# janstenner/DistributedConvRL-PDE-Control

Measured on AMD Instinct MI355X. Metric: env-steps/sec (KS CNAB2 env step + conv actor fwd + DDPG fwd/bwd/update), higher is better.
Workload: dtype f32

## Files before the change

distributedconvrl-pde-control_amd/_lib.py:

```python
import ctypes as C
import os

_HERE = os.path.dirname(os.path.abspath(__file__))
LIB_PATH = os.environ.get("PDEC_LIB_PATH") or os.path.join(_HERE, "libpdeconv.so")

PDEC_F32, PDEC_F64 = 0, 1
PDE_KS_CNAB2, PDE_KSEG_RK4, PDE_KS_RK4_FD, PDE_FLUID_RK4, PDE_KSEG2D_RK4 = 0, 1, 2, 3, 4
ACT_IDENTITY, ACT_RELU, ACT_TANH = 0, 1, 2

Handle = C.c_uint64


class PdecError(RuntimeError):
    pass


class EnvCfg(C.Structure):
    _fields_ = [
        ("pde_kind", C.c_int), ("dtype", C.c_int), ("B", C.c_int), ("N", C.c_int),
        ("n_species", C.c_int), ("S", C.c_int), ("A", C.c_int), ("window", C.c_int),
        ("temporal_steps", C.c_int), ("mono", C.c_int), ("K", C.c_int), ("check_max_value", C.c_int),
        ("Lx", C.c_double), ("dt", C.c_double), ("mu", C.c_double), ("max_value", C.c_double),
        ("sensor_scale", C.c_double), ("agent_power", C.c_double), ("reward_in_scale", C.c_double),
        ("reward_offset", C.c_double), ("reward_power", C.c_double), ("reward_denom", C.c_double),
# ... 99 lines not shown
    "pdec_ledger_eval_close": [Handle, _vp, _vp, _i64, _i64, _i64],
    "pdec_ledger_eval_read": [Handle, _vp, _vp, _vp, _vp], "pdec_ledger_eval_best": [Handle, _pd, C.POINTER(_i64)],
    "pdec_ledger_eval_best_params": [Handle, Handle],
    "pdec_epclock_create": [C.POINTER(Handle), Handle, _i, _i, _i, _u64, _i, _i], "pdec_epclock_set": [Handle, _vp],
    "pdec_epclock_step": [Handle] + [_vp] * 9, "pdec_epclock_read": [Handle, _vp, _vp, _vp, _vp, _vp],
    "pdec_nstep_create": [C.POINTER(Handle), _i, _i, _i, _i, _i],
    "pdec_nstep_step": [Handle, _vp, _vp, _vp, _vp, _d, _vp, _vp, _vp, _vp], "pdec_nstep_read": [Handle, C.POINTER(_i64)] + [_vp] * 4,
    "pdec_telemetry_create": [C.POINTER(Handle), _i, _i, _i, _i, _i, _i, Handle, Handle],
    "pdec_telemetry_step": [Handle, _vp, _vp, _vp, _vp, _vp, _d], "pdec_telemetry_update": [Handle] * 5 + [_vp],
    "pdec_telemetry_read": [Handle, _vp, C.POINTER(_i64), _vp, C.POINTER(_i64), _vp], "pdec_telemetry_reset": [Handle],
    "pdec_capture_begin": [Handle], "pdec_capture_end": [Handle, C.POINTER(Handle)],
    "pdec_graph_launch": [Handle, _vp], "pdec_graph_num_nodes": [Handle, C.POINTER(_i)],
    "pdec_event_create": [C.POINTER(Handle)], "pdec_event_record": [Handle, _vp], "pdec_stream_wait_event": [_vp, Handle], "pdec_mlp_set_stop_event": [Handle, Handle], "pdec_mlp_flush_stop_event": [Handle],
    "pdec_mlp_set_reduce_event": [Handle, Handle],
    "pdec_env_set_simd_sharing": [Handle, C.c_int, C.POINTER(C.c_int)],
    "pdec_ddpg_critic_grads": [Handle] * 4 + [_vp] * 5 + [_i, _d, _i, _d, _vp],
    "pdec_ddpg_actor_grads": [Handle, Handle, _vp, _i, _d, _vp],
    "pdec_ddpg_update": [Handle] * 4 + [_vp] * 5 + [_i, _d, _d, _i, _d, _d, _pd, _pd],
    "pdec_comm_unique_id": [_vp], "pdec_comm_create": [C.POINTER(Handle), _i, _i, _vp],
    "pdec_comm_create_timeout": [C.POINTER(Handle), _i, _i, _vp, _i],
    "pdec_allreduce_grads": [Handle, Handle], "pdec_allreduce": [Handle, _vp, _sz, _i, _vp],
    "pdec_allreduce_grads_on": [Handle, Handle, _vp],
}
DEBUG_SIGNATURES = {
    "pdec_debug_wave_fft": [_vp, _vp, _i, _i, _i],
    "pdec_debug_wave_fft_f32": [_vp, _vp, _i, _i, _i],
    "pdec_debug_critic_stamps": [Handle, _i, _pd],
    "pdec_debug_fused_image": [Handle, _i, _vp] + [C.POINTER(_i)] * 4,
    "pdec_debug_kseg2d_probe": [Handle, _i, _i, _i, _pd],
    "pdec_debug_spin_us": [_vp, _d],
# ... 150 lines not shown
```

distributedconvrl-pde-control_amd/csrc/env.hip:

```cpp
#include "env_sense.hpp"
#include "roll_actor.hpp"

namespace pdec {

template <class T, int MODE, bool FLT = false>
__global__ void sense_kernel(EnvArg<T, FLT> e, const T* __restrict__ y, const T* __restrict__ action,
                             const T* __restrict__ action_prev, const T* __restrict__ state_prev,
                             T* __restrict__ out) {
  sense_traj<T, MODE, FLT>(e, blockIdx.x, y, action, action_prev, state_prev, out);
}

template <class T>
__global__ void terminal_from_done_kernel(const int32_t* __restrict__ done, int B, int cpt, T* __restrict__ term) {
  const int i = blockIdx.x * blockDim.x + threadIdx.x;
  if (i < B * cpt) term[i] = (done[i / cpt] & 1) ? (T)1 : (T)0;
}

static int launch_step(Env& E, int mode, const StepArgs& a) {
  const pdec_env_cfg& c = E.cfg;
  const bool fused = mode == 0;
  const LaunchSync sync = E.sync;
  E.sync = LaunchSync{};
  if (sync.wait || sync.done) {
    const bool ok = c.pde_kind == PDEC_PDE_KS_CNAB2 && fused && c.B <= 2 && !E.member && c.dtype == PDEC_F64 && ks_is_fixed_plan(E.engine) &&
// ... 265 lines not shown
  }

int pdec_env_set_terminal_out(pdec_handle h, void* terminal_per_column) {
  GET_ENV(E, h);
  E->term_out = terminal_per_column;
  return PDEC_OK;
}

int pdec_env_set_simd_sharing(pdec_handle h, int on, int* effective) {
  GET_ENV(E, h);
  E->share_simd = on != 0;
  if (effective) *effective = (E->share_simd && E->cfg.pde_kind == PDEC_PDE_KS_CNAB2 && ks_is_single_wave(E->engine) && E->cfg.dtype == PDEC_F32) ? 1 : 0;
  return PDEC_OK;
}

int pdec_env_set_member_layout(pdec_handle h, int on) {
  GET_ENV(E, h);
  const int k = E->cfg.pde_kind;
  PDEC_REQUIRE(!on || k == PDEC_PDE_KS_CNAB2 || k == PDEC_PDE_KSEG_RK4,
               "pdec_env_set_member_layout: the 1-D KS and Keller-Segel environments only (pde kind %d)", k);
  PDEC_REQUIRE(!on || !E->rsum_out, "pdec_env_set_member_layout: per-pair reward partials are set (pdec_env_set_reward_partials_out)");
  E->member = on != 0;
  return PDEC_OK;
}

int pdec_env_set_disturbance(pdec_handle h, const void* mu_per_trajectory) {
  GET_ENV(E, h);
  const pdec_env_cfg& c = E->cfg;
  if (mu_per_trajectory) {
    PDEC_REQUIRE(c.pde_kind != PDEC_PDE_FLUID_RK4, "pdec_env_set_disturbance: the fluid has no disturbance term (KS environments only)");
// ... 174 lines not shown
```

distributedconvrl-pde-control_amd/csrc/env.hpp:

```cpp
#pragma once
#include "common.hpp"
#include "fft_lds.hpp"
#include <type_traits>

namespace pdec {

template <class T>
struct EnvDev {
  int B, N, S, A, ns, window, temporal, mono, K, check_max, n_species, rk2, prio;
  int mem, na;
  T sensor_scale, agent_power, r_in_scale, r_offset, r_power, r_denom, a_pun, da_pun, max_value;
  T dx, hstep, dist_mu;
  const T* Gs;
  const int* sn0;
  const T* GaC;
  const int* an0;
  int Wd, Cnt;
  float* rsum_out;
  T* term_out;
  const T* gsum;
  const int* a2s;
  const int* fmap;
  const T *c1, *c2, *c3, *c4, *g;
  const C2<T>* dhat;
// ... 13 lines not shown
struct EnvDevF : EnvDev<T> {
  FaultDev<T> flt;
};
template <class T, bool FLT>
using EnvArg = std::conditional_t<FLT, EnvDevF<T>, EnvDev<T>>;

enum class KsEngine {
  Wave256,
  Wave1024,
  LdsR4_256,
  LdsR4_1024,
  Fixed192,
  Fixed240,
  Fixed600,
  Generic,
};
constexpr bool ks_is_single_wave(KsEngine k) { return k == KsEngine::Wave256; }
constexpr bool ks_is_fixed_plan(KsEngine k) { return k == KsEngine::Fixed192 || k == KsEngine::Fixed240 || k == KsEngine::Fixed600; }
inline KsEngine ks_pick_engine(int N, bool force_generic, bool lds_fft) {
  if (force_generic) return KsEngine::Generic;
  if (N == 256) return lds_fft ? KsEngine::LdsR4_256 : KsEngine::Wave256;
  if (N == 1024) return lds_fft ? KsEngine::LdsR4_1024 : KsEngine::Wave1024;
  return N == 192 ? KsEngine::Fixed192 : N == 240 ? KsEngine::Fixed240 : N == 600 ? KsEngine::Fixed600 : KsEngine::Generic;
}
int ks_engine_threads(KsEngine k);

struct StepArgs {
  const void *y_in, *p, *action, *action_prev, *state_prev;
  void *y_out, *p_out, *state_out, *reward_out;
  int32_t* done;
};

struct Env : Object {
  pdec_env_cfg cfg;
  DevBuf Gs, sn0, GaC, an0, gsum, a2s, fmap, c1, c2, c3, c4, g, dhat, dhat1, tw;
  int Wd = 0, Cnt = 0;
  DevBuf stage;
  DevBuf roll;
  DevBuf roll_tab;
  std::vector<const void*> roll_tab_host;
  DevBuf mem_scratch;
  void* term_out = nullptr;
  float* rsum_out = nullptr;
  bool share_simd = false;
  bool member = false;
  const void* mu_b = nullptr;
  int control_from = 0;
  const void *act_gain = nullptr, *sens_gain = nullptr, *sens_bias = nullptr;
  bool faults() const { return act_gain || sens_gain || sens_bias; }
  FftPlan fft;
  int nthreads = 64;
  KsEngine engine = KsEngine::Generic;
  size_t lds_bytes = 0;
  Env() : Object(Kind::Env) {}
  virtual int part_streams() const { return 0; }
  virtual int set_part_streams(const hipStream_t*, int) { return PDEC_OK; }
  virtual int actuate(const void* action, void* p_out);
  virtual int featurize(const void* y, const void* state_prev, void* state_out, const void* action = nullptr);
  virtual int reward(const void* y, const void* action, const void* action_prev, void* r_out);
  virtual int pde_step(const void* y_in, const void* p, void* y_out, int32_t* done);
  virtual int rhs_eval(const void* y, const void* p, void* out);
  virtual int env_step(const StepArgs& a);
};

template <class T>
EnvDev<T> make_dev(const Env& E) {
  const pdec_env_cfg& c = E.cfg;
  EnvDev<T> e;
  e.B = c.B; e.N = c.N; e.S = c.S; e.A = c.A; e.window = c.window; e.temporal = c.temporal_steps;
  e.mono = c.mono; e.K = c.K; e.check_max = c.check_max_value; e.n_species = c.n_species;
  e.mem = c.memory_size; e.na = 1 + c.memory_size;
  e.ns = c.mono ? c.S : c.window * c.n_species * c.temporal_steps + c.memory_size;
  e.sensor_scale = (T)c.sensor_scale; e.agent_power = (T)c.agent_power;
  e.r_in_scale = (T)c.reward_in_scale; e.r_offset = (T)c.reward_offset; e.r_power = (T)c.reward_power;
  e.r_denom = (T)c.reward_denom; e.a_pun = (T)c.action_punish; e.da_pun = (T)c.delta_action_punish;
  e.max_value = (T)c.max_value;
  e.dx = (T)(c.Lx / c.N);
  e.hstep = (T)(c.dt / c.K);
// ... 92 lines not shown
```

distributedconvrl-pde-control_amd/csrc/env_sense.hpp:

```cpp
#pragma once
#include "env.hpp"

namespace pdec {


template <class T, class YF>
__device__ __forceinline__ void sense_dots(const EnvDev<T>& e, YF yf, T* dots, T* part, int tid, int nt) {
  const int S = e.S, N = e.N, Wd = e.Wd;
  int ng = nt / S;
  if (ng < 1) ng = 1;
  if (ng > 8) ng = 8;
  const int chunk = (Wd + ng - 1) / ng;
  for (int idx = tid; idx < ng * S; idx += nt) {
    const int grp = idx / S, s = idx - grp * S;
    int j0 = grp * chunk, j1 = j0 + chunk;
    if (j1 > Wd) j1 = Wd;
    int n = e.sn0[s] + j0;
    if (n >= N) n -= N;
    T p0[4] = {0, 0, 0, 0}, p1[4] = {0, 0, 0, 0};
    int j = j0;
    for (; j + 8 <= j1; j += 8) {
      T gk[8];
#pragma unroll
      for (int u = 0; u < 8; ++u) gk[u] = e.Gs[(size_t)(j + u) * S + s];
// ... 325 lines not shown
```

distributedconvrl-pde-control_amd/csrc/ks_engines.hpp:

```cpp
#pragma once
#include "env.hpp"

namespace pdec {

#define KS_MPT 4

template <class T>
struct FftGeneric {
  static constexpr int kThreads = 1024;
  C2<T>*X, *Y;
  const C2<T>* tw;
  FftPlan pl;
  int N, tid, nt;
  __device__ __forceinline__ void init(unsigned char* smem, const EnvDev<T>& e, int tid_, int nt_) {
    N = e.N; tid = tid_; nt = nt_; pl = e.fft;
    X = reinterpret_cast<C2<T>*>(smem);
    Y = X + N;
    C2<T>* t = Y + N;
    for (int k = tid; k < N; k += nt) t[k] = e.tw[k];
    tw = t;
  }
  static __host__ __device__ size_t lds_complex(int N) { return 3 * (size_t)N; }
  __device__ __forceinline__ int mode_index(int j) const { return tid + j * nt; }
  __device__ __forceinline__ int phys_index(int j) const { return tid + j * nt; }
// ... 276 lines not shown
      dft4<+1>(a);
      exchange<2>(a); twiddle<2, +1>(a); dft4<+1>(a);
      exchange<1>(a); twiddle<1, +1>(a); dft4<+1>(a);
      exchange<0>(a); twiddle<0, +1>(a); dft4<+1>(a);
    }
  }
  __device__ __forceinline__ C2<T>* publish(const C2<T> (&a)[KS_MPT]) {
    __syncthreads();
#pragma unroll
    for (int j = 0; j < 4; ++j) buf[tid + NT * j] = a[j];
    __syncthreads();
    return buf;
  }
};

template <class T>
struct FftWave1024 {
  static constexpr int kThreads = 256;
  static constexpr int N = 1024, NT = 256;
  FftWave256<T> core;
  C2<T>* buf[2];
  C2<T> wx[3];
  int tid, lane, wv, par;
  __device__ __forceinline__ void init(unsigned char* smem, const EnvDev<T>& e, int tid_, int) {
    tid = tid_; lane = tid & 63; wv = tid >> 6; par = 0;
    buf[0] = reinterpret_cast<C2<T>*>(smem);
    buf[1] = buf[0] + N;
    core.tid = lane;
    core.b1 = (lane & 2) != 0; core.b0 = (lane & 1) != 0;
    core.buf = buf[0];
// ... 122 lines not shown
  __device__ __forceinline__ C2<T>* publish(const C2<T> (&a)[KS_MPT]) {
    __syncthreads();
#pragma unroll
    for (int j = 0; j < KS_MPT; ++j) {
      const int k = phys_index(j);
      if (k < N) buf[0][k] = a[j];
    }
    __syncthreads();
    return buf[0];
  }
};
template <class T> using FftFixed192 = FftFixed<T, 192, 4, 4, 4, 3, 4, 1>;
template <class T> using FftFixed240 = FftFixed<T, 240, 4, 4, 5, 3, 4, 1>;
template <class T> using FftFixed600 = FftFixed<T, 600, 5, 4, 5, 5, 2, 3>;

template <KsEngine K, class ENG> struct KsEngineTag { static constexpr KsEngine kind = K; using type = ENG; };
template <class T, class F>
auto with_ks_engine(KsEngine k, F&& f) {
  switch (k) {
    case KsEngine::Wave256: return f(KsEngineTag<KsEngine::Wave256, FftWave256<T>>{});
    case KsEngine::Wave1024: return f(KsEngineTag<KsEngine::Wave1024, FftWave1024<T>>{});
    case KsEngine::LdsR4_256: return f(KsEngineTag<KsEngine::LdsR4_256, FftR4<T, 4>>{});
    case KsEngine::LdsR4_1024: return f(KsEngineTag<KsEngine::LdsR4_1024, FftR4<T, 5>>{});
    case KsEngine::Fixed192: return f(KsEngineTag<KsEngine::Fixed192, FftFixed192<T>>{});
    case KsEngine::Fixed240: return f(KsEngineTag<KsEngine::Fixed240, FftFixed240<T>>{});
    case KsEngine::Fixed600: return f(KsEngineTag<KsEngine::Fixed600, FftFixed600<T>>{});
    default: return f(KsEngineTag<KsEngine::Generic, FftGeneric<T>>{});
  }
}

}
```

distributedconvrl-pde-control_amd/csrc/ks_step.hip:

```cpp
#include "env_sense.hpp"
#include "ks_engines.hpp"

namespace pdec {

template <class T, class ENG, bool FUSED, bool SHARE = false, bool SYNC = false, bool MU = false, bool FLT = false>
__global__ void __launch_bounds__(ENG::kThreads, SHARE ? 8 : 1) ks_env_step_kernel(EnvArg<T, FLT> e, const T* __restrict__ y_in, const T* __restrict__ p_in,
                                   const T* __restrict__ action, const T* __restrict__ action_prev,
                                   const T* __restrict__ state_prev, T* __restrict__ y_out,
                                   T* __restrict__ p_out, T* __restrict__ state_out,
                                   T* __restrict__ reward_out, int32_t* __restrict__ done) {
  extern __shared__ __align__(16) unsigned char smem_raw[];
  const int N = e.N, tid = threadIdx.x, nt = blockDim.x;
  if constexpr (SYNC) launch_sync_wait(e.sync);
  set_wave_prio(e.prio);
  ENG eng;
  eng.init(smem_raw, e, tid, nt);
  T* act = reinterpret_cast<T*>(reinterpret_cast<C2<T>*>(smem_raw) + ENG::lds_complex(N));
  T* actp = act + 2 * e.A;
  T* dots = actp + 2 * e.A;
  T* part = dots + 2 * e.S;
  T* red = part + 16 * e.S;

  const int b0 = e.member ? (int)blockIdx.x : 2 * (int)blockIdx.x, b1 = b0 + 1;
  const bool has1 = !e.member && b1 < e.B;
  const size_t o0 = (size_t)b0 * N, o1 = (size_t)b1 * N;
  const C2<T>* __restrict__ dtab = MU ? e.dhat1 : e.dhat;
  T m0 = 1, m1 = 1;
// ... 4 lines not shown
      act[a] = action[(size_t)b0 * e.A + a];
      act[e.A + a] = has1 ? action[(size_t)b1 * e.A + a] : (T)0;
      actp[a] = action_prev[(size_t)b0 * e.A + a];
      actp[e.A + a] = has1 ? action_prev[(size_t)b1 * e.A + a] : (T)0;
      if constexpr (FLT) {
        act[a] = fault_action<T>(e.flt, b0, e.A, a, act[a]);
        if (has1) act[e.A + a] = fault_action<T>(e.flt, b1, e.A, a, act[e.A + a]);
      }
    }
  }
  __syncthreads();

  constexpr bool LDSC = SHARE;
  typedef T T4v __attribute__((ext_vector_type(4)));
  T4v* cst = reinterpret_cast<T4v*>(smem_raw + ((size_t)(reinterpret_cast<unsigned char*>(red + 16) - smem_raw + 15) & ~(size_t)15));
  C2<T> U[KS_MPT], Nn[KS_MPT], Ck[KS_MPT], v[KS_MPT];
  T kc1[KS_MPT], kc2[KS_MPT], kc3[KS_MPT], kg[KS_MPT];
  T pa4[KS_MPT], pb4[KS_MPT];
  if (FUSED) {
    int n4[KS_MPT];
#pragma unroll
    for (int j = 0; j < KS_MPT; ++j) n4[j] = eng.phys_index(j);
    if ((N & 3) == 0 && 2 * N <= 16 * e.S) {
      actuate_consecutive<T>(e, act, act + e.A, part, tid, nt);
#pragma unroll
      for (int j = 0; j < KS_MPT; ++j) {
        pa4[j] = n4[j] < N ? part[n4[j]] : (T)0;
        pb4[j] = n4[j] < N ? part[N + n4[j]] : (T)0;
      }
    } else {
      actuate_cells<T, KS_MPT>(e, act, act + e.A, n4, pa4, pb4);
    }
    if constexpr (FLT) {
      __syncthreads();
      for (int a = tid; a < e.A; a += nt) {
        act[a] = action[(size_t)b0 * e.A + a];
        if (has1) act[e.A + a] = action[(size_t)b1 * e.A + a];
      }
    }
  }
#pragma unroll
  for (int j = 0; j < KS_MPT; ++j) {
    const int n = eng.phys_index(j);
    T pa = 0, pb = 0;
    if (n < N) {
      if (FUSED) {
        pa = pa4[j]; pb = pb4[j];
        if (!has1) pb = 0;
        if (p_out) {
          p_out[o0 + n] = pa;
          if (has1) p_out[o1 + n] = pb;
        }
      } else {
        pa = p_in[o0 + n];
        pb = has1 ? p_in[o1 + n] : (T)0;
      }
    }
    v[j] = mk<T>(pa, pb);
  }
  eng.template run<-1>(v);
#pragma unroll
  for (int j = 0; j < KS_MPT; ++j) {
    const int k = eng.mode_index(j);
    if (k < N) {
      const C2<T> d = dtab[k];
      const T c4 = e.c4[k];
      if constexpr (MU) Ck[j] = mk<T>(c4 * v[j].x + (m0 * d.x - m1 * d.y), c4 * v[j].y + (m0 * d.y + m1 * d.x));
      else Ck[j] = mk<T>(c4 * v[j].x + (d.x - d.y), c4 * v[j].y + (d.x + d.y));
      kc1[j] = e.c1[k];
      kc2[j] = e.c2[k];
      kc3[j] = e.c3[k];
      kg[j] = e.g[k];
    } else {
      Ck[j] = mk<T>(0, 0);
      kc1[j] = kc2[j] = kc3[j] = kg[j] = 0;
    }
    if constexpr (LDSC) cst[j * nt + tid] = T4v{kc1[j], kc2[j], kc3[j], kg[j]};
  }
  if constexpr (LDSC) {
    cst[4 * nt + tid] = T4v{Ck[0].x, Ck[0].y, Ck[1].x, Ck[1].y};
    cst[5 * nt + tid] = T4v{Ck[2].x, Ck[2].y, Ck[3].x, Ck[3].y};
  }
#pragma unroll
  for (int j = 0; j < KS_MPT; ++j) {
    const int n = eng.phys_index(j);
    U[j] = n < N ? mk<T>(y_in[o0 + n], has1 ? y_in[o1 + n] : (T)0) : mk<T>(0, 0);
    v[j] = mk<T>(U[j].x * U[j].x, U[j].y * U[j].y);
  }
  eng.template run<-1>(v);
#pragma unroll
  for (int j = 0; j < KS_MPT; ++j) Nn[j] = cscale(mul_i<+1, T>(v[j]), kg[j]);
  if constexpr (LDSC) {
    cst[6 * nt + tid] = T4v{Nn[0].x, Nn[0].y, Nn[1].x, Nn[1].y};
    cst[7 * nt + tid] = T4v{Nn[2].x, Nn[2].y, Nn[3].x, Nn[3].y};
  }
  eng.template run<-1>(U);
  const T invN = (T)1 / (T)N;
  if constexpr (LDSC) {
    for (int it = 0; it < e.K; ++it) {
#pragma unroll
      for (int j = 0; j < KS_MPT; ++j) v[j] = U[j];
      eng.template run<+1>(v);
#pragma unroll
      for (int j = 0; j < KS_MPT; ++j) {
        const T wr = v[j].x * invN, wi = v[j].y * invN;
        v[j] = mk<T>(wr * wr, wi * wi);
      }
      eng.template run<-1>(v);
#pragma unroll
      for (int h = 0; h < 2; ++h) {
        const T4v nn = cst[(6 + h) * nt + tid], ck = cst[(4 + h) * nt + tid];
        T4v nw;
#pragma unroll
        for (int u = 0; u < 2; ++u) {
          const int j = 2 * h + u;
          const T4v c = cst[j * nt + tid];
          const C2<T> n1 = cscale(mul_i<+1, T>(v[j]), c[3]);
          U[j] = mk<T>(c[0] * U[j].x + c[1] * n1.x - c[2] * nn[2 * u] + ck[2 * u],
                       c[0] * U[j].y + c[1] * n1.y - c[2] * nn[2 * u + 1] + ck[2 * u + 1]);
          nw[2 * u] = n1.x; nw[2 * u + 1] = n1.y;
        }
        cst[(6 + h) * nt + tid] = nw;
      }
    }
  } else {
    for (int it = 0; it < e.K; ++it) {
#pragma unroll
      for (int j = 0; j < KS_MPT; ++j) v[j] = U[j];
      eng.template run<+1>(v);
#pragma unroll
      for (int j = 0; j < KS_MPT; ++j) {
        const T wr = v[j].x * invN, wi = v[j].y * invN;
        v[j] = mk<T>(wr * wr, wi * wi);
      }
      eng.template run<-1>(v);
#pragma unroll
      for (int j = 0; j < KS_MPT; ++j) {
        const C2<T> nn1 = Nn[j];
        Nn[j] = cscale(mul_i<+1, T>(v[j]), kg[j]);
        U[j] = mk<T>(kc1[j] * U[j].x + kc2[j] * Nn[j].x - kc3[j] * nn1.x + Ck[j].x,
                     kc1[j] * U[j].y + kc2[j] * Nn[j].y - kc3[j] * nn1.y + Ck[j].y);
      }
    }
  }
  eng.template run<+1>(U);
  T mx0 = 0, mx1 = 0;
#pragma unroll
  for (int j = 0; j < KS_MPT; ++j) {
    const int n = eng.phys_index(j);
    U[j] = mk<T>(U[j].x * invN, U[j].y * invN);
    if (n < N) {
      y_out[o0 + n] = U[j].x;
      if (has1) y_out[o1 + n] = U[j].y;
      if (!(fabs(U[j].x) <= e.max_value)) mx0 = 1;
      if (!(fabs(U[j].y) <= e.max_value)) mx1 = 1;
    }
  }
  if (done) {
    mx0 = block_max<T>(mx0, red, tid, nt);
    mx1 = block_max<T>(mx1, red, tid, nt);
    if (tid == 0) {
      const bool chk = e.check_max == 1;
      done[b0] = (chk && mx0 > 0) ? 1 : 0;
      if (has1) done[b1] = (chk && mx1 > 0) ? 1 : 0;
    }
    if (FUSED && e.check_max != 2) {
      write_terminal<T>(e, b0, e.check_max == 1 && mx0 > 0, tid, nt);
      if (has1) write_terminal<T>(e, b1, e.check_max == 1 && mx1 > 0, tid, nt);
    }
  }
  if (!FUSED) return;
  const T* Rt = reinterpret_cast<const T*>(eng.publish(U));
  sense_dots<T>(e, [&](int r, int n) { return Rt[2 * n + r]; }, dots, part, tid, nt);
  const int rw = e.mono ? 1 : e.A;
  const int sw = e.mono ? e.S : e.A * e.ns;
  T rmine;
  const T* fd = dots;
  if constexpr (FLT) {
    fault_dots<T>(e.flt, b0, e.S, dots, part, tid, nt);
    if (has1) fault_dots<T>(e.flt, b1, e.S, dots + e.S, part + e.S, tid, nt);
    __syncthreads();
    fd = part;
  }
  if (e.fmap && !e.mono) {
    rmine = reward_pair<T>(e, dots, dots + e.S, act, act + e.A, actp, actp + e.A, reward_out + (size_t)b0 * rw,
                           has1 ? reward_out + (size_t)b1 * rw : nullptr, tid, nt);
    featurize_pair<T>(e, fd, fd + e.S, state_out + (size_t)b0 * sw, has1 ? state_out + (size_t)b1 * sw : nullptr, tid, nt);
  } else {
    rmine = reward_traj<T>(e, dots, act, actp, reward_out + (size_t)b0 * rw, tid, nt);
    featurize_traj<T>(e, fd, state_prev ? state_prev + (size_t)b0 * sw : nullptr, state_out + (size_t)b0 * sw, tid, nt);
    if (has1) {
      rmine += reward_traj<T>(e, dots + e.S, act + e.A, actp + e.A, reward_out + (size_t)b1 * rw, tid, nt);
      featurize_traj<T>(e, fd + e.S, state_prev ? state_prev + (size_t)b1 * sw : nullptr,
                        state_out + (size_t)b1 * sw, tid, nt);
    }
  }
  if (e.rsum_out) {
    float v = (float)rmine;
    for (int off = 32; off > 0; off >>= 1) v += __shfl_xor(v, off);
    __syncthreads();
    if ((tid & 63) == 0) red[tid >> 6] = (T)v;
    __syncthreads();
    if (tid == 0) {
      float tot = 0.f;
      for (int i = 0; i < (nt + 63) / 64; ++i) tot += (float)red[i];
      e.rsum_out[blockIdx.x] = tot;
    }
// ... 3 lines not shown
    if (tid == 0) {
      for (int t = 0; t < (has1 ? 2 : 1); ++t) {
        T m = 0;
        const T* r = reward_out + (size_t)(b0 + t) * rw;
        for (int a = 0; a < rw; ++a)
          if (!(fabs(r[a]) <= e.max_value)) m = 1;
        done[b0 + t] = m > 0 ? 1 : 0;
        write_terminal<T>(e, b0 + t, m > 0, 0, 1);
      }
    }
  }
  if constexpr (SYNC) launch_sync_done(e.sync);
}

int ks_engine_threads(KsEngine k) {
  return with_ks_engine<float>(k, [](auto tag) { return (int)decltype(tag)::type::kThreads; });
}
size_t ks_lds_bytes(const pdec_env_cfg& c, KsEngine k) {
  const size_t fft = with_ks_engine<float>(k, [&](auto tag) { return decltype(tag)::type::lds_complex(c.N); });
  return (fft * 2 + 4 * (size_t)c.A + 2 * c.S + 16 * c.S + 16) * dtype_size(c.dtype);
}

template <class T, class ENG, KsEngine KIND, bool FLT>
auto ks_step_kernel_for(bool fused, bool share, bool synced, bool mu) {
  auto kern = mu ? ks_env_step_kernel<T, ENG, true, false, false, true, FLT> : ks_env_step_kernel<T, ENG, true, false, false, false, FLT>;
  if constexpr (!FLT)
    if (!fused) kern = mu ? ks_env_step_kernel<T, ENG, false, false, false, true> : ks_env_step_kernel<T, ENG, false>;
  if constexpr (sizeof(T) == 4 && ks_is_single_wave(KIND))
    if (share) kern = mu ? ks_env_step_kernel<T, ENG, true, true, false, true, FLT> : ks_env_step_kernel<T, ENG, true, true, false, false, FLT>;
  if constexpr (!FLT && sizeof(T) == 8 && ks_is_fixed_plan(KIND))
    if (synced) kern = mu ? ks_env_step_kernel<T, ENG, true, false, true, true> : ks_env_step_kernel<T, ENG, true, false, true>;
  return kern;
}

int ks_launch_step(Env& E, bool fused, const StepArgs& a, const LaunchSync& sync) {
  const pdec_env_cfg& c = E.cfg;
  const dim3 grid(E.member ? c.B : (c.B + 1) / 2), block(E.nthreads);
  const bool synced = sync.wait || sync.done;
  const bool mu = E.mu_b != nullptr;
  const bool share = fused && E.share_simd && c.dtype == PDEC_F32 && ks_is_single_wave(E.engine);
  const size_t lds = E.lds_bytes + (share ? 16 + 8 * 16 * 64 : 0);
  const bool timed = c.dtype == PDEC_F32 && ks_is_single_wave(E.engine) && fused && E.prof && E.prof_reps == 1;
  by_dtype(c.dtype, [&](auto t) {
    using T = decltype(t);
    with_ks_engine<T>(E.engine, [&](auto tag) {
      using ENG = typename decltype(tag)::type;
      constexpr KsEngine KIND = decltype(tag)::kind;
      auto launch = [&](auto kern, const auto& e) {
        if (timed) {
          PDEC_TIMED_LAUNCH(&E, "ks_env_step", kern, grid, block, lds, PDEC_STEP_KERNEL_ARGS(T, e, a));
          return;
        }
        ProfScope ps(&E, fused ? "ks_env_step" : "ks_pde_step", !synced && a.y_out != a.y_in && a.state_out != a.state_prev);
        for (int rep = 0; rep < ps.reps; ++rep) hipLaunchKernelGGL(kern, grid, block, lds, E.stream, PDEC_STEP_KERNEL_ARGS(T, e, a));
      };
      if (fused && E.faults()) {
        launch(ks_step_kernel_for<T, ENG, KIND, true>(fused, share, synced, mu), make_dev_faults<T>(E));
      } else {
        EnvDev<T> e = make_dev<T>(E);
        e.sync = sync;
        launch(ks_step_kernel_for<T, ENG, KIND, false>(fused, share, synced, mu), e);
      }
    });
  });
  PDEC_HIP(hipGetLastError());
  return PDEC_OK;
}

}
```

distributedconvrl-pde-control_amd/env.py:

```python
import ctypes as C

import numpy as np
import torch

from . import _lib


def _stream_ptr(stream):
    if stream is None:
        return None
    return C.c_void_p(stream.cuda_stream)


_FAST_STREAM_SWITCH = hasattr(torch._C, "_cuda_getCurrentStream") and hasattr(torch._C, "_cuda_setStream")


class _on_stream:
    __slots__ = ("s", "prev", "ctx")

    def __init__(self, stream):
        self.s, self.prev, self.ctx = stream, None, None

    def __enter__(self):
        s = self.s
# ... 290 lines not shown
        self.time += self.dt
        self._done_stale = True
        if self.autoreset:
            own_action = self.action.data_ptr() not in self._adopted
            _lib.check(self.lib.pdec_env_autoreset(
                self._h, _lib.ptr(self._done_flags), _lib.ptr(self.y), _lib.ptr(self.y0), _lib.ptr(self.state),
                _lib.ptr(self._state0), _lib.ptr(self.action) if own_action else None,
                _lib.ptr(self.action0) if own_action else None, _lib.ptr(self.reward)))

    def set_simd_sharing(self, on=True):
        import ctypes as C
        eff = C.c_int()
        _lib.check(self.lib.pdec_env_set_simd_sharing(self.handle, 1 if on else 0, C.byref(eff)))
        return bool(eff.value)

    def set_disturbance(self, mu):
        if mu is None:
            _lib.check(self.lib.pdec_env_set_disturbance(self._h, None))
            self.mu = None
            return
        with _on_stream(self.stream):
            t = mu if isinstance(mu, torch.Tensor) else torch.as_tensor(np.array(mu, dtype=np.float64, copy=True))
            if t.dim() != 1 or int(t.shape[0]) != self.B:
                raise _lib.PdecError(f"PDEenv.set_disturbance: expected {self.B} amplitudes (one per trajectory), got shape "
                                     f"{tuple(t.shape)}")
            t = t.to(device=self.device, dtype=self.dtype).contiguous().clone()
        _lib.check(self.lib.pdec_env_set_disturbance(self._h, _lib.ptr(t)))
        self.mu = t

    def set_faults(self, actuator_gain=None, sensor_gain=None, sensor_bias=None):
# ... 98 lines not shown
```

distributedconvrl-pde-control_amd/pipeline.py:

```python
import copy
import ctypes as C
import os
from types import SimpleNamespace

import torch

from . import _lib
from .pipeline_episodes import check_episode_mode, setup_episodes
from .pipeline_eval import Evaluation, check_eval_args, eval_score
from .pipeline_nstep import NStep, check_n_step, gamma_n
from .pipeline_replay import Replay
from .pipeline_telemetry import (TELEMETRY_STEP_COLUMNS, TELEMETRY_UPDATE_COLUMNS, Telemetry, check_telemetry,
                                 ring_columns)

PERIOD = 6


class _Event(_lib.Owned):

    def __init__(self, lib):
        super().__init__(lib)
        _lib.check(lib.pdec_event_create(C.byref(self.h)))

    def record(self, stream):
# ... 121 lines not shown
        self.actor = self.policy.behavior_actor.model
        yes = C.c_int()
        _lib.check(self.lib.pdec_mlp_acts_on_published_copy(self.actor.handle, C.byref(yes)))
        self.act_in_place = not bool(yes.value)
        self.kick_env_after_critic = ((not self.act_in_place and not self.use_replay) if kick_env_after_critic is None
                                      else bool(kick_env_after_critic))
        if os.environ.get("PDEC_KICK") in ("0", "1"):
            self.kick_env_after_critic = os.environ["PDEC_KICK"] == "1"
        self.stop_events = (self.rpart is not None and Ev is _Event and not self.serial
                            and os.environ.get("PDEC_STOP_EVENTS", "1") != "0")
        self.simd_sharing = False
        if not self.serial and self.rpart is not None and os.environ.get("PDEC_SHARE", "0") == "1":
            eff = C.c_int()
            _lib.check(self.lib.pdec_env_set_simd_sharing(env.handle, 1, C.byref(eff)))
            self.simd_sharing = bool(eff.value)
        self.graphs = {}
        self._progs = {}
        aliases = (self.policy.behavior_critic.model.dtype == torch.float32) if self.use_replay else self._batch_aliases
        self.fast_eager = os.environ.get("PDEC_FAST_EAGER", "1") == "1" and Ev is _Event and aliases
        self._key, self._captured = None, False
        self.n_graph_launches = self.n_eager_steps = 0
        self.noise_scale = None
        self.set_noise_scale(noise_scale)
        self.noise_ab = self.noise_state = None
        self.set_noise_corr(noise_corr)
        self.nstep = NStep(self) if self.n_step > 1 else None
        self._telem = Telemetry(self) if self.telemetry_capacity > 0 else None
        self.replay = Replay(self) if self.use_replay else None
        self.ledger, self.inits, self.clock = setup_episodes(self, log_episodes, min_best_episode, random_init, init_seed, init_rng,
                                                             init_rank)
# ... 551 lines not shown
    def telemetry_reset(self):
        self._on("_telem", "TrainPipeline.telemetry_reset: telemetry is off (telemetry=0)").reset()

    def sync(self):
        self._flush_actor_finish()
        for s in (self.s_env, self.s_upd, self.s_ar, self.s_eval):
            if s is not None:
                s.synchronize()

    def close(self):
        if self.s_eval is not None:
            self.s_eval.synchronize()
        if getattr(self, "simd_sharing", False):
            self.lib.pdec_env_set_simd_sharing(self.env.handle, 0, None)
            self.simd_sharing = False
        self._drop_graphs()
```

include/pdeconv.h:

```cpp
#ifndef PDECONV_H
#define PDECONV_H

#include <stddef.h>
#include <stdint.h>

#ifdef __cplusplus
extern "C" {
#endif

typedef uint64_t pdec_handle;

enum { PDEC_F32 = 0, PDEC_F64 = 1 };

enum {
  PDEC_OK = 0,
  PDEC_E_INVALID = -1,
  PDEC_E_HIP = -2,
  PDEC_E_HANDLE = -3,
  PDEC_E_NOGPU = -4,
  PDEC_E_COMM = -5
};

enum {
  PDEC_PDE_KS_CNAB2 = 0,
// ... 156 lines not shown
                     double* actor_loss, double* critic_loss);

int pdec_ddpg_update_async(pdec_handle A, pdec_handle C, pdec_handle At, pdec_handle Ct,
                           const void* s, const void* a, const void* r, const void* t, const void* snext,
                           int Bu, double gamma, double rho, int quirk, double eta_actor, double eta_critic,
                           void* losses_dev);

int pdec_ddpg_update_small(pdec_handle A, pdec_handle C, pdec_handle At, pdec_handle Ct,
                           const void* state_trace, const void* action_trace, const void* reward_trace,
                           const void* terminal_trace, const int32_t* idx_s, const int32_t* idx_rt,
                           const int32_t* idx_sn, int loops, int Bu, double gamma, double rho, int quirk,
                           double eta_actor, double eta_critic, void* losses_dev);

int pdec_reward_mean(pdec_handle any_handle, const void* r, int n, void* mean_out);
int pdec_env_set_simd_sharing(pdec_handle env, int on, int* effective);
int pdec_env_set_reward_partials_out(pdec_handle env, void* partial_sums, int* n_partials);
int pdec_env_part_streams(pdec_handle env, int* n);
int pdec_env_set_part_streams(pdec_handle env, void* const* hip_streams, int n);
int pdec_ddpg_set_reward_partials(pdec_handle critic, const void* partial_sums, int n);
int pdec_ddpg_set_reward_mean(pdec_handle critic, const void* mean_dev);

int pdec_ddpg_set_reward_groups(pdec_handle critic, int g, int L);

int pdec_ddpg_update_small_rng(pdec_handle A, pdec_handle C, pdec_handle At, pdec_handle Ct,
                               const void* state_trace, const void* action_trace, const void* reward_trace,
                               const void* terminal_trace, int loops, int Bu, uint64_t seed, uint64_t offset,
                               int64_t n_valid, int64_t n_rt, int64_t capacity, int stride, double gamma, double rho,
                               int quirk, double eta_actor, double eta_critic, void* losses_dev);

int pdec_ddpg_update_critic_async(pdec_handle A, pdec_handle C, pdec_handle At, pdec_handle Ct,
// ... 114 lines not shown
```

Before: 4.933 million.

## Add two-wave 256-point FFT engine for the fused KS CNAB2 env step

Adds a new FFT engine, Wave256x2, that splits the 256-point KS FFT across two wavefronts of 64 lanes (128 threads, 2 modes per thread). One butterfly level exchanges data across the two waves through LDS with a barrier, and the remaining levels use intra-wave DPP and permlane swaps. It is enabled by default in the pipeline for the fused f32 step when SIMD sharing is off. Reward and sense reductions are limited to the first 64 threads. The aim is to halve per-thread register work and the serial FFT latency of each env-step block, at the cost of extra LDS round trips and cross-wave barriers inside every FFT.

```diff
diff --git a/distributedconvrl-pde-control_amd/_lib.py b/distributedconvrl-pde-control_amd/_lib.py
--- a/distributedconvrl-pde-control_amd/_lib.py
+++ b/distributedconvrl-pde-control_amd/_lib.py
@@ -137,6 +137,7 @@
     "pdec_event_create": [C.POINTER(Handle)], "pdec_event_record": [Handle, _vp], "pdec_stream_wait_event": [_vp, Handle], "pdec_mlp_set_stop_event": [Handle, Handle], "pdec_mlp_flush_stop_event": [Handle],
     "pdec_mlp_set_reduce_event": [Handle, Handle],
     "pdec_env_set_simd_sharing": [Handle, C.c_int, C.POINTER(C.c_int)],
+    "pdec_env_set_two_wave_step": [Handle, C.c_int, C.POINTER(C.c_int)],
     "pdec_ddpg_critic_grads": [Handle] * 4 + [_vp] * 5 + [_i, _d, _i, _d, _vp],
     "pdec_ddpg_actor_grads": [Handle, Handle, _vp, _i, _d, _vp],
     "pdec_ddpg_update": [Handle] * 4 + [_vp] * 5 + [_i, _d, _d, _i, _d, _d, _pd, _pd],
diff --git a/distributedconvrl-pde-control_amd/csrc/env.hip b/distributedconvrl-pde-control_amd/csrc/env.hip
--- a/distributedconvrl-pde-control_amd/csrc/env.hip
+++ b/distributedconvrl-pde-control_amd/csrc/env.hip
@@ -303,6 +303,13 @@
   return PDEC_OK;
 }
 
+int pdec_env_set_two_wave_step(pdec_handle h, int on, int* effective) {
+  GET_ENV(E, h);
+  E->two_wave = on != 0;
+  if (effective) *effective = ks_step_engine(*E, true) == KsEngine::Wave256x2 ? 1 : 0;
+  return PDEC_OK;
+}
+
 int pdec_env_set_member_layout(pdec_handle h, int on) {
   GET_ENV(E, h);
   const int k = E->cfg.pde_kind;
diff --git a/distributedconvrl-pde-control_amd/csrc/env.hpp b/distributedconvrl-pde-control_amd/csrc/env.hpp
--- a/distributedconvrl-pde-control_amd/csrc/env.hpp
+++ b/distributedconvrl-pde-control_amd/csrc/env.hpp
@@ -51,6 +51,7 @@
   Fixed240,
   Fixed600,
   Generic,
+  Wave256x2,
 };
 constexpr bool ks_is_single_wave(KsEngine k) { return k == KsEngine::Wave256; }
 constexpr bool ks_is_fixed_plan(KsEngine k) { return k == KsEngine::Fixed192 || k == KsEngine::Fixed240 || k == KsEngine::Fixed600; }
@@ -80,6 +81,7 @@
   void* term_out = nullptr;
   float* rsum_out = nullptr;
   bool share_simd = false;
+  bool two_wave = false;
   bool member = false;
   const void* mu_b = nullptr;
   int control_from = 0;
@@ -99,6 +101,12 @@
   virtual int rhs_eval(const void* y, const void* p, void* out);
   virtual int env_step(const StepArgs& a);
 };
+
+inline KsEngine ks_step_engine(const Env& E, bool fused) {
+  const bool two = E.two_wave && fused && E.cfg.pde_kind == PDEC_PDE_KS_CNAB2 && E.engine == KsEngine::Wave256 &&
+                   E.cfg.dtype == PDEC_F32 && !E.share_simd && !E.member && !E.mu_b && !E.faults();
+  return two ? KsEngine::Wave256x2 : E.engine;
+}
 
 template <class T>
 EnvDev<T> make_dev(const Env& E) {
diff --git a/distributedconvrl-pde-control_amd/csrc/env_sense.hpp b/distributedconvrl-pde-control_amd/csrc/env_sense.hpp
--- a/distributedconvrl-pde-control_amd/csrc/env_sense.hpp
+++ b/distributedconvrl-pde-control_amd/csrc/env_sense.hpp
@@ -3,6 +3,7 @@
 
 namespace pdec {
 
+constexpr int SUM_IDLE_TID = 1 << 28;
 
 template <class T, class YF>
 __device__ __forceinline__ void sense_dots(const EnvDev<T>& e, YF yf, T* dots, T* part, int tid, int nt) {
diff --git a/distributedconvrl-pde-control_amd/csrc/ks_engines.hpp b/distributedconvrl-pde-control_amd/csrc/ks_engines.hpp
--- a/distributedconvrl-pde-control_amd/csrc/ks_engines.hpp
+++ b/distributedconvrl-pde-control_amd/csrc/ks_engines.hpp
@@ -314,6 +314,158 @@
   }
 };
 
+__device__ __forceinline__ void wave_pair_barrier() { asm volatile("s_waitcnt lgkmcnt(0)\n\ts_barrier" ::: "memory"); }
+#define PDEC_XSTEP2(CA, CB, MASK, P0, Q0, P1, Q1)                                                          \
+  {                                                                                                        \
+    float n0_, n1_;                                                                                        \
+    asm("s_nop 1\n\t"                                                                                      \
+        "s_mov_b64 vcc, %6\n\t"                                                                            \
+        "v_cndmask_b32_dpp %4, %0, %1, vcc " CA " row_mask:0xf bank_mask:0xf\n\t"                           \
+        "v_cndmask_b32_dpp %5, %2, %3, vcc " CA " row_mask:0xf bank_mask:0xf\n\t"                           \
+        "s_mov_b64 vcc, %7\n\t"                                                                            \
+        "v_cndmask_b32_dpp %0, %1, %0, vcc " CB " row_mask:0xf bank_mask:0xf\n\t"                           \
+        "v_cndmask_b32_dpp %2, %3, %2, vcc " CB " row_mask:0xf bank_mask:0xf"                                \
+        : "+v"(P0), "+v"(Q0), "+v"(P1), "+v"(Q1), "=&v"(n0_), "=&v"(n1_)                                   \
+        : "s"(MASK), "s"(~(MASK))                                                                          \
+        : "vcc");                                                                                          \
+    Q0 = n0_; Q1 = n1_;                                                                                    \
+  }
+template <int SGN>
+__device__ __forceinline__ pkf2 pk_cmul_lanes(pkf2 a, pkf2 w, unsigned long long mask) {
+  pkf2 t;
+  unsigned long long sv;
+  if (SGN < 0)
+    asm("s_and_saveexec_b64 %2, %4\n\t"
+        "v_pk_mul_f32 %1, %0, %3 op_sel_hi:[1,0]\n\t"
+        "v_pk_fma_f32 %0, %0, %3, %1 op_sel:[1,1,0] op_sel_hi:[0,1,1] neg_lo:[0,1,0]\n\t"
+        "s_mov_b64 exec, %2"
+        : "+v"(a), "=&v"(t), "=&s"(sv) : "v"(w), "s"(mask) : "scc");
+  else
+    asm("s_and_saveexec_b64 %2, %4\n\t"
+        "v_pk_mul_f32 %1, %0, %3 op_sel_hi:[1,0]\n\t"
+        "v_pk_fma_f32 %0, %0, %3, %1 op_sel:[1,1,0] op_sel_hi:[0,1,1] neg_hi:[0,1,0]\n\t"
+        "s_mov_b64 exec, %2"
+        : "+v"(a), "=&v"(t), "=&s"(sv) : "v"(w), "s"(mask) : "scc");
+  return a;
+}
+
+struct FftWave256x2 {
+  static constexpr int kThreads = 128;
+  static constexpr int kMpt = 2;
+  static constexpr int kSumThreads = 64;
+  static constexpr int N = 256, NT = 128;
+  C2<float>* buf;
+  pkf2 w0[3], w1[3];
+  int tid, lane, wv, par;
+  __device__ __forceinline__ void init(unsigned char* smem, const EnvDev<float>& e, int tid_, int) {
+    tid = tid_; lane = tid & 63; par = 0;
+    wv = __builtin_amdgcn_readfirstlane(tid >> 6);
+    buf = reinterpret_cast<C2<float>*>(smem);
+    const int kl[3] = {wv, (lane >> 4) & 1, (lane >> 2) & 1};
+    const int low[3] = {lane, 4 * (lane & 15), 16 * (lane & 3)};
+#pragma unroll
+    for (int st = 0; st < 3; ++st) {
+      w0[st] = __builtin_bit_cast(pkf2, e.tw[(kl[st] * low[st]) & 255]);
+      w1[st] = __builtin_bit_cast(pkf2, e.tw[((kl[st] + 2) * low[st]) & 255]);
+    }
+  }
+  static __host__ __device__ size_t lds_complex(int) { return (size_t)N; }
+  __device__ __forceinline__ int mode_index(int j) const {
+    const int k0 = wv + 2 * (lane >> 5), k1 = ((lane >> 4) & 1) + 2 * ((lane >> 3) & 1);
+    const int k2 = ((lane >> 2) & 1) + 2 * ((lane >> 1) & 1), k3 = (lane & 1) + 2 * j;
+    return k0 + 4 * k1 + 16 * k2 + 64 * k3;
+  }
+  __device__ __forceinline__ int phys_index(int j) const { return tid + NT * j; }
+
+  static __device__ __forceinline__ void level1(C2<float> (&a)[2]) {
+    const pkf2 p = __builtin_bit_cast(pkf2, a[0]), q = __builtin_bit_cast(pkf2, a[1]);
+    a[0] = __builtin_bit_cast(C2<float>, p + q);
+    a[1] = __builtin_bit_cast(C2<float>, p - q);
+  }
+  template <int SGN>
+  static __device__ __forceinline__ void level2(C2<float> (&a)[2], bool d) {
+    const C2<float> b = a[1];
+    pkf2 r;
+    if (SGN < 0) { r.x = d ? b.y : b.x; r.y = d ? -b.x : b.y; }
+    else { r.x = d ? -b.y : b.x; r.y = d ? b.x : b.y; }
+    const pkf2 p = __builtin_bit_cast(pkf2, a[0]);
+    a[0] = __builtin_bit_cast(C2<float>, p + r);
+    a[1] = __builtin_bit_cast(C2<float>, p - r);
+  }
+  template <int SGN>
+  __device__ __forceinline__ void level2_wave(C2<float> (&a)[2]) const {
+    const pkf2 p = __builtin_bit_cast(pkf2, a[0]), q = __builtin_bit_cast(pkf2, a[1]);
+    if (wv) {
+      a[0] = __builtin_bit_cast(C2<float>, SGN < 0 ? pk_add_mi(p, q) : pk_add_pi(p, q));
+      a[1] = __builtin_bit_cast(C2<float>, SGN < 0 ? pk_add_pi(p, q) : pk_add_mi(p, q));
+    } else {
+      a[0] = __builtin_bit_cast(C2<float>, p + q);
+      a[1] = __builtin_bit_cast(C2<float>, p - q);
+    }
+  }
+  template <int ST, int SGN>
+  __device__ __forceinline__ void twiddle(C2<float> (&a)[2]) const {
+    a[1] = __builtin_bit_cast(C2<float>, pk_cmul<SGN>(__builtin_bit_cast(pkf2, a[1]), w1[ST]));
+    if (ST == 0) {
+      if (wv) a[0] = __builtin_bit_cast(C2<float>, pk_cmul<SGN>(__builtin_bit_cast(pkf2, a[0]), w0[0]));
+    } else {
+      a[0] = __builtin_bit_cast(C2<float>, pk_cmul_lanes<SGN>(__builtin_bit_cast(pkf2, a[0]), w0[ST],
+                                                              ST == 1 ? 0xFFFF0000FFFF0000ull : 0xF0F0F0F0F0F0F0F0ull));
+    }
+  }
+  template <int BIT>
+  static __device__ __forceinline__ void xch(C2<float> (&a)[2]) {
+    if (BIT == 5) {
+      asm("s_nop 1\n\t"
+          "v_permlane32_swap_b32 %0, %2\n\t"
+          "v_permlane32_swap_b32 %1, %3"
+          : "+v"(a[0].x), "+v"(a[0].y), "+v"(a[1].x), "+v"(a[1].y));
+    } else if (BIT == 4) {
+      asm("s_nop 1\n\t"
+          "v_permlane16_swap_b32 %0, %2\n\t"
+          "v_permlane16_swap_b32 %1, %3"
+          : "+v"(a[0].x), "+v"(a[0].y), "+v"(a[1].x), "+v"(a[1].y));
+    } else if (BIT == 3) {
+      PDEC_XSTEP2("row_ror:8", "row_ror:8", 0xFF00FF00FF00FF00ull, a[0].x, a[1].x, a[0].y, a[1].y)
+    } else if (BIT == 2) {
+      PDEC_XSTEP2("row_ror:12", "row_ror:4", 0xF0F0F0F0F0F0F0F0ull, a[0].x, a[1].x, a[0].y, a[1].y)
+    } else if (BIT == 1) {
+      PDEC_XSTEP2("quad_perm:[2,3,0,1]", "quad_perm:[2,3,0,1]", 0xCCCCCCCCCCCCCCCCull, a[0].x, a[1].x, a[0].y, a[1].y)
+    } else {
+      PDEC_XSTEP2("quad_perm:[1,0,3,2]", "quad_perm:[1,0,3,2]", 0xAAAAAAAAAAAAAAAAull, a[0].x, a[1].x, a[0].y, a[1].y)
+    }
+  }
+  __device__ __forceinline__ void xch_wave(C2<float> (&a)[2]) {
+    C2<float>* X = buf + 128 * par;
+    par ^= 1;
+    if (wv) X[tid] = a[0]; else X[tid] = a[1];
+    wave_pair_barrier();
+    if (wv) a[0] = X[tid ^ 64]; else a[1] = X[tid ^ 64];
+  }
+  template <int SGN>
+  __device__ __forceinline__ void run(C2<float> (&a)[2]) {
+    const bool d4 = (lane & 16) != 0, d2 = (lane & 4) != 0, d0 = (lane & 1) != 0;
+    if (SGN < 0) {
+      level1(a); xch_wave(a); level2_wave<-1>(a); twiddle<0, -1>(a);
+      xch<5>(a); level1(a); xch<4>(a); level2<-1>(a, d4); twiddle<1, -1>(a);
+      xch<3>(a); level1(a); xch<2>(a); level2<-1>(a, d2); twiddle<2, -1>(a);
+      xch<1>(a); level1(a); xch<0>(a); level2<-1>(a, d0);
+    } else {
+      level1(a); xch<0>(a); level2<+1>(a, d0);
+      xch<1>(a); twiddle<2, +1>(a); level1(a); xch<2>(a); level2<+1>(a, d2);
+      xch<3>(a); twiddle<1, +1>(a); level1(a); xch<4>(a); level2<+1>(a, d4);
+      xch<5>(a); twiddle<0, +1>(a); level1(a); xch_wave(a); level2_wave<+1>(a);
+    }
+  }
+  __device__ __forceinline__ C2<float>* publish(const C2<float> (&a)[2]) {
+    __syncthreads();
+#pragma unroll
+    for (int j = 0; j < 2; ++j) buf[tid + NT * j] = a[j];
+    __syncthreads();
+    return buf;
+  }
+};
+
 template <class T>
 struct FftWave1024 {
   static constexpr int kThreads = 256;
@@ -466,9 +618,16 @@
 template <class T> using FftFixed240 = FftFixed<T, 240, 4, 4, 5, 3, 4, 1>;
 template <class T> using FftFixed600 = FftFixed<T, 600, 5, 4, 5, 5, 2, 3>;
 
+template <class ENG, class = void> struct KsMpt { static constexpr int value = KS_MPT; };
+template <class ENG> struct KsMpt<ENG, std::void_t<decltype(ENG::kMpt)>> { static constexpr int value = ENG::kMpt; };
+template <class ENG, class = void> struct KsSumThreads { static constexpr int value = 0; };
+template <class ENG> struct KsSumThreads<ENG, std::void_t<decltype(ENG::kSumThreads)>> { static constexpr int value = ENG::kSumThreads; };
+
 template <KsEngine K, class ENG> struct KsEngineTag { static constexpr KsEngine kind = K; using type = ENG; };
-template <class T, class F>
+template <class T, bool STEP = false, class F>
 auto with_ks_engine(KsEngine k, F&& f) {
+  if constexpr (STEP && sizeof(T) == 4)
+    if (k == KsEngine::Wave256x2) return f(KsEngineTag<KsEngine::Wave256x2, FftWave256x2>{});
   switch (k) {
     case KsEngine::Wave256: return f(KsEngineTag<KsEngine::Wave256, FftWave256<T>>{});
     case KsEngine::Wave1024: return f(KsEngineTag<KsEngine::Wave1024, FftWave1024<T>>{});
diff --git a/distributedconvrl-pde-control_amd/csrc/ks_step.hip b/distributedconvrl-pde-control_amd/csrc/ks_step.hip
--- a/distributedconvrl-pde-control_amd/csrc/ks_step.hip
+++ b/distributedconvrl-pde-control_amd/csrc/ks_step.hip
@@ -11,6 +11,9 @@
                                    T* __restrict__ reward_out, int32_t* __restrict__ done) {
   extern __shared__ __align__(16) unsigned char smem_raw[];
   const int N = e.N, tid = threadIdx.x, nt = blockDim.x;
+  constexpr int MPT = KsMpt<ENG>::value;
+  constexpr int SUMT = KsSumThreads<ENG>::value;
+  const int stid = SUMT ? (tid < SUMT ? tid : SUM_IDLE_TID) : tid, snt = SUMT ? SUMT : nt;
   if constexpr (SYNC) launch_sync_wait(e.sync);
   set_wave_prio(e.prio);
   ENG eng;
@@ -45,22 +48,22 @@
   constexpr bool LDSC = SHARE;
   typedef T T4v __attribute__((ext_vector_type(4)));
   T4v* cst = reinterpret_cast<T4v*>(smem_raw + ((size_t)(reinterpret_cast<unsigned char*>(red + 16) - smem_raw + 15) & ~(size_t)15));
-  C2<T> U[KS_MPT], Nn[KS_MPT], Ck[KS_MPT], v[KS_MPT];
-  T kc1[KS_MPT], kc2[KS_MPT], kc3[KS_MPT], kg[KS_MPT];
-  T pa4[KS_MPT], pb4[KS_MPT];
+  C2<T> U[MPT], Nn[MPT], Ck[MPT], v[MPT];
+  T kc1[MPT], kc2[MPT], kc3[MPT], kg[MPT];
+  T pa4[MPT], pb4[MPT];
   if (FUSED) {
-    int n4[KS_MPT];
-#pragma unroll
-    for (int j = 0; j < KS_MPT; ++j) n4[j] = eng.phys_index(j);
+    int n4[MPT];
+#pragma unroll
+    for (int j = 0; j < MPT; ++j) n4[j] = eng.phys_index(j);
     if ((N & 3) == 0 && 2 * N <= 16 * e.S) {
       actuate_consecutive<T>(e, act, act + e.A, part, tid, nt);
 #pragma unroll
-      for (int j = 0; j < KS_MPT; ++j) {
+      for (int j = 0; j < MPT; ++j) {
         pa4[j] = n4[j] < N ? part[n4[j]] : (T)0;
         pb4[j] = n4[j] < N ? part[N + n4[j]] : (T)0;
       }
     } else {
-      actuate_cells<T, KS_MPT>(e, act, act + e.A, n4, pa4, pb4);
+      actuate_cells<T, MPT>(e, act, act + e.A, n4, pa4, pb4);
     }
     if constexpr (FLT) {
       __syncthreads();
@@ -71,7 +74,7 @@
     }
   }
 #pragma unroll
-  for (int j = 0; j < KS_MPT; ++j) {
+  for (int j = 0; j < MPT; ++j) {
     const int n = eng.phys_index(j);
     T pa = 0, pb = 0;
     if (n < N) {
@@ -91,7 +94,7 @@
   }
   eng.template run<-1>(v);
 #pragma unroll
-  for (int j = 0; j < KS_MPT; ++j) {
+  for (int j = 0; j < MPT; ++j) {
     const int k = eng.mode_index(j);
     if (k < N) {
       const C2<T> d = dtab[k];
@@ -113,14 +116,14 @@
     cst[5 * nt + tid] = T4v{Ck[2].x, Ck[2].y, Ck[3].x, Ck[3].y};
   }
 #pragma unroll
-  for (int j = 0; j < KS_MPT; ++j) {
+  for (int j = 0; j < MPT; ++j) {
     const int n = eng.phys_index(j);
     U[j] = n < N ? mk<T>(y_in[o0 + n], has1 ? y_in[o1 + n] : (T)0) : mk<T>(0, 0);
     v[j] = mk<T>(U[j].x * U[j].x, U[j].y * U[j].y);
   }
   eng.template run<-1>(v);
 #pragma unroll
-  for (int j = 0; j < KS_MPT; ++j) Nn[j] = cscale(mul_i<+1, T>(v[j]), kg[j]);
+  for (int j = 0; j < MPT; ++j) Nn[j] = cscale(mul_i<+1, T>(v[j]), kg[j]);
   if constexpr (LDSC) {
     cst[6 * nt + tid] = T4v{Nn[0].x, Nn[0].y, Nn[1].x, Nn[1].y};
     cst[7 * nt + tid] = T4v{Nn[2].x, Nn[2].y, Nn[3].x, Nn[3].y};
@@ -130,10 +133,10 @@
   if constexpr (LDSC) {
     for (int it = 0; it < e.K; ++it) {
 #pragma unroll
-      for (int j = 0; j < KS_MPT; ++j) v[j] = U[j];
+      for (int j = 0; j < MPT; ++j) v[j] = U[j];
       eng.template run<+1>(v);
 #pragma unroll
-      for (int j = 0; j < KS_MPT; ++j) {
+      for (int j = 0; j < MPT; ++j) {
         const T wr = v[j].x * invN, wi = v[j].y * invN;
         v[j] = mk<T>(wr * wr, wi * wi);
       }
@@ -157,16 +160,16 @@
   } else {
     for (int it = 0; it < e.K; ++it) {
 #pragma unroll
-      for (int j = 0; j < KS_MPT; ++j) v[j] = U[j];
+      for (int j = 0; j < MPT; ++j) v[j] = U[j];
       eng.template run<+1>(v);
 #pragma unroll
-      for (int j = 0; j < KS_MPT; ++j) {
+      for (int j = 0; j < MPT; ++j) {
         const T wr = v[j].x * invN, wi = v[j].y * invN;
         v[j] = mk<T>(wr * wr, wi * wi);
       }
       eng.template run<-1>(v);
 #pragma unroll
-      for (int j = 0; j < KS_MPT; ++j) {
+      for (int j = 0; j < MPT; ++j) {
         const C2<T> nn1 = Nn[j];
         Nn[j] = cscale(mul_i<+1, T>(v[j]), kg[j]);
         U[j] = mk<T>(kc1[j] * U[j].x + kc2[j] * Nn[j].x - kc3[j] * nn1.x + Ck[j].x,
@@ -177,7 +180,7 @@
   eng.template run<+1>(U);
   T mx0 = 0, mx1 = 0;
 #pragma unroll
-  for (int j = 0; j < KS_MPT; ++j) {
+  for (int j = 0; j < MPT; ++j) {
     const int n = eng.phys_index(j);
     U[j] = mk<T>(U[j].x * invN, U[j].y * invN);
     if (n < N) {
@@ -202,7 +205,7 @@
   }
   if (!FUSED) return;
   const T* Rt = reinterpret_cast<const T*>(eng.publish(U));
-  sense_dots<T>(e, [&](int r, int n) { return Rt[2 * n + r]; }, dots, part, tid, nt);
+  sense_dots<T>(e, [&](int r, int n) { return Rt[2 * n + r]; }, dots, part, stid, snt);
   const int rw = e.mono ? 1 : e.A;
   const int sw = e.mono ? e.S : e.A * e.ns;
   T rmine;
@@ -215,13 +218,13 @@
   }
   if (e.fmap && !e.mono) {
     rmine = reward_pair<T>(e, dots, dots + e.S, act, act + e.A, actp, actp + e.A, reward_out + (size_t)b0 * rw,
-                           has1 ? reward_out + (size_t)b1 * rw : nullptr, tid, nt);
+                           has1 ? reward_out + (size_t)b1 * rw : nullptr, stid, snt);
     featurize_pair<T>(e, fd, fd + e.S, state_out + (size_t)b0 * sw, has1 ? state_out + (size_t)b1 * sw : nullptr, tid, nt);
   } else {
-    rmine = reward_traj<T>(e, dots, act, actp, reward_out + (size_t)b0 * rw, tid, nt);
+    rmine = reward_traj<T>(e, dots, act, actp, reward_out + (size_t)b0 * rw, stid, snt);
     featurize_traj<T>(e, fd, state_prev ? state_prev + (size_t)b0 * sw : nullptr, state_out + (size_t)b0 * sw, tid, nt);
     if (has1) {
-      rmine += reward_traj<T>(e, dots + e.S, act + e.A, actp + e.A, reward_out + (size_t)b1 * rw, tid, nt);
+      rmine += reward_traj<T>(e, dots + e.S, act + e.A, actp + e.A, reward_out + (size_t)b1 * rw, stid, snt);
       featurize_traj<T>(e, fd + e.S, state_prev ? state_prev + (size_t)b1 * sw : nullptr,
                         state_out + (size_t)b1 * sw, tid, nt);
     }
@@ -255,10 +258,10 @@
 }
 
 int ks_engine_threads(KsEngine k) {
-  return with_ks_engine<float>(k, [](auto tag) { return (int)decltype(tag)::type::kThreads; });
+  return with_ks_engine<float, true>(k, [](auto tag) { return (int)decltype(tag)::type::kThreads; });
 }
 size_t ks_lds_bytes(const pdec_env_cfg& c, KsEngine k) {
-  const size_t fft = with_ks_engine<float>(k, [&](auto tag) { return decltype(tag)::type::lds_complex(c.N); });
+  const size_t fft = with_ks_engine<float, true>(k, [&](auto tag) { return decltype(tag)::type::lds_complex(c.N); });
   return (fft * 2 + 4 * (size_t)c.A + 2 * c.S + 16 * c.S + 16) * dtype_size(c.dtype);
 }
 
@@ -276,15 +279,17 @@
 
 int ks_launch_step(Env& E, bool fused, const StepArgs& a, const LaunchSync& sync) {
   const pdec_env_cfg& c = E.cfg;
-  const dim3 grid(E.member ? c.B : (c.B + 1) / 2), block(E.nthreads);
+  const KsEngine engine = ks_step_engine(E, fused);
+  const bool two = engine != E.engine;
+  const dim3 grid(E.member ? c.B : (c.B + 1) / 2), block(two ? ks_engine_threads(engine) : E.nthreads);
   const bool synced = sync.wait || sync.done;
   const bool mu = E.mu_b != nullptr;
   const bool share = fused && E.share_simd && c.dtype == PDEC_F32 && ks_is_single_wave(E.engine);
-  const size_t lds = E.lds_bytes + (share ? 16 + 8 * 16 * 64 : 0);
+  const size_t lds = (two ? ks_lds_bytes(c, engine) : E.lds_bytes) + (share ? 16 + 8 * 16 * 64 : 0);
   const bool timed = c.dtype == PDEC_F32 && ks_is_single_wave(E.engine) && fused && E.prof && E.prof_reps == 1;
   by_dtype(c.dtype, [&](auto t) {
     using T = decltype(t);
-    with_ks_engine<T>(E.engine, [&](auto tag) {
+    with_ks_engine<T, true>(engine, [&](auto tag) {
       using ENG = typename decltype(tag)::type;
       constexpr KsEngine KIND = decltype(tag)::kind;
       auto launch = [&](auto kern, const auto& e) {
@@ -295,7 +300,11 @@
         ProfScope ps(&E, fused ? "ks_env_step" : "ks_pde_step", !synced && a.y_out != a.y_in && a.state_out != a.state_prev);
         for (int rep = 0; rep < ps.reps; ++rep) hipLaunchKernelGGL(kern, grid, block, lds, E.stream, PDEC_STEP_KERNEL_ARGS(T, e, a));
       };
-      if (fused && E.faults()) {
+      if constexpr (KIND == KsEngine::Wave256x2) {
+        EnvDev<T> e = make_dev<T>(E);
+        e.sync = sync;
+        launch(ks_env_step_kernel<T, ENG, true>, e);
+      } else if (fused && E.faults()) {
         launch(ks_step_kernel_for<T, ENG, KIND, true>(fused, share, synced, mu), make_dev_faults<T>(E));
       } else {
         EnvDev<T> e = make_dev<T>(E);
diff --git a/distributedconvrl-pde-control_amd/env.py b/distributedconvrl-pde-control_amd/env.py
--- a/distributedconvrl-pde-control_amd/env.py
+++ b/distributedconvrl-pde-control_amd/env.py
@@ -328,6 +328,12 @@
         _lib.check(self.lib.pdec_env_set_simd_sharing(self.handle, 1 if on else 0, C.byref(eff)))
         return bool(eff.value)
 
+    def set_two_wave_step(self, on=True):
+        import ctypes as C
+        eff = C.c_int()
+        _lib.check(self.lib.pdec_env_set_two_wave_step(self.handle, 1 if on else 0, C.byref(eff)))
+        return bool(eff.value)
+
     def set_disturbance(self, mu):
         if mu is None:
             _lib.check(self.lib.pdec_env_set_disturbance(self._h, None))
diff --git a/distributedconvrl-pde-control_amd/pipeline.py b/distributedconvrl-pde-control_amd/pipeline.py
--- a/distributedconvrl-pde-control_amd/pipeline.py
+++ b/distributedconvrl-pde-control_amd/pipeline.py
@@ -159,6 +159,12 @@
             eff = C.c_int()
             _lib.check(self.lib.pdec_env_set_simd_sharing(env.handle, 1, C.byref(eff)))
             self.simd_sharing = bool(eff.value)
+        self.two_wave = False
+        if (not self.serial and self.rpart is not None and not self.simd_sharing
+                and os.environ.get("PDEC_TWO_WAVE", "1") != "0"):
+            eff = C.c_int()
+            _lib.check(self.lib.pdec_env_set_two_wave_step(env.handle, 1, C.byref(eff)))
+            self.two_wave = bool(eff.value)
         self.graphs = {}
         self._progs = {}
         aliases = (self.policy.behavior_critic.model.dtype == torch.float32) if self.use_replay else self._batch_aliases
@@ -740,4 +746,7 @@
         if getattr(self, "simd_sharing", False):
             self.lib.pdec_env_set_simd_sharing(self.env.handle, 0, None)
             self.simd_sharing = False
+        if getattr(self, "two_wave", False):
+            self.lib.pdec_env_set_two_wave_step(self.env.handle, 0, None)
+            self.two_wave = False
         self._drop_graphs()
diff --git a/include/pdeconv.h b/include/pdeconv.h
--- a/include/pdeconv.h
+++ b/include/pdeconv.h
@@ -194,6 +194,7 @@
 
 int pdec_reward_mean(pdec_handle any_handle, const void* r, int n, void* mean_out);
 int pdec_env_set_simd_sharing(pdec_handle env, int on, int* effective);
+int pdec_env_set_two_wave_step(pdec_handle env, int on, int* effective);
 int pdec_env_set_reward_partials_out(pdec_handle env, void* partial_sums, int* n_partials);
 int pdec_env_part_streams(pdec_handle env, int* n);
 int pdec_env_set_part_streams(pdec_handle env, void* const* hip_streams, int n);
```

Measured after the change: 5.021 million (median of 6 runs). +1.8%, better.
